# billamiable/MultiCol-SLAM-Annotation

Hardware: AMD Instinct MI355X
Metric: kfeatures/sec + LocalBA iters/sec, 3×754×480 fisheye, 1/2/4/8 MI355X (higher is better)
Workload: dtype u8; 1 GPU; config B: 3-cam Lafida rig 754x480, 2000 feat/cam, extract + consecutive-multi-frame top-2 Hamming match; parallelism=dp1 (independent multi-frame segments)

## Files before the change

multicol-slam-annotation_amd/csrc/extractor.hip:

```cpp
#include "host_util.hpp"
#include "extractor_plan.hpp"
#include "extractor_kernels.hpp"
#include "pyr_units.hpp"
#include <algorithm>
#include <cstdlib>
#include <cstring>
#include <new>
#include <vector>

namespace mcs {

template <typename T>
static int dalloc(T** p, size_t count, size_t pad_bytes = 256) {
  *p = nullptr;
  MCS_HIP_CHECK(hipMalloc((void**)p, count * sizeof(T) + pad_bytes));
  return MCS_OK;
}

}

struct mcs_extractor {
  mcs::Plan plan;
  int device = 0;
  int max_frames = 0;
  int32_t* d_xofs = nullptr; int16_t* d_alpha = nullptr;
  int32_t* d_yofs = nullptr; int16_t* d_beta = nullptr;
  mcs::CellDesc* d_cells = nullptr;
  mcs::FastUnit* d_units = nullptr;
  uint8_t* d_pyr = nullptr;
  uint8_t* d_blur = nullptr;
  uint32_t* d_slots = nullptr;
  int32_t* d_cell_counts = nullptr;
  uint32_t* d_cand = nullptr;
  int32_t* d_cnode = nullptr;
  uint32_t* d_sel = nullptr;
  int32_t* d_sel_count = nullptr;
  uint8_t* d_mask_pyr = nullptr; int n_masks = 0;
  mcs::FastUnit* d_munits = nullptr; int64_t munit_stride = 0;
  uint8_t* d_mask_single = nullptr;
  struct PyrTable {
    int fclass = 0; bool masked = false;
    mcs::PyrUnit* d_units = nullptr; int64_t mstride = 0;
    int32_t off[mcs::kMaxLevels] = {}, n[mcs::kMaxLevels] = {};
  };
  std::vector<PyrTable> pyr_tabs;
  std::vector<mcs::PyrNeed> pyr_need;
  uint8_t* d_in = nullptr;
  mcs_keypoint* d_kps = nullptr; uint8_t* d_desc = nullptr; int32_t* d_count = nullptr;
  uint8_t* d_dmask = nullptr;
  mcs_cam_model* d_cams = nullptr; int n_cams = 0;
  hipStream_t side = nullptr; hipEvent_t ev_fork = nullptr, ev_join = nullptr;
  const uint8_t* last_img0 = nullptr;
  int last_frames = 0;
  static constexpr int kRing = 256;
  bool timing = false;
  hipEvent_t* ev = nullptr;
  int ev_count = 0;
};

namespace mcs {

static void fill_level_ptrs(const Plan& pl, LevelPtrs& lp) {
  for (int l = 0; l < kMaxLevels; l++) {
    const bool v = l < pl.nlevels;
    lp.w[l] = v ? pl.lv[l].w : 0; lp.h[l] = v ? pl.lv[l].h : 0;
    lp.pitch[l] = v ? pl.lv[l].pitch : 0; lp.bpitch[l] = v ? pl.lv[l].bpitch : 0;
    lp.pyr_off[l] = v ? pl.lv[l].pyr_off : 0; lp.img_off[l] = v ? pl.lv[l].img_off : 0;
    lp.mask_off[l] = v ? pl.lv[l].mask_off : 0;
  }
}

// ... 14 lines not shown
      lists[(size_t)m * kMaxLevels + l].swap(lv[l]);
    }
  }
  int64_t stride = 0;
  for (int l = 0; l < pl.nlevels; l++) { t.off[l] = (int32_t)stride; stride += t.n[l]; }
  stride = std::max<int64_t>(stride, 1);
  std::vector<PyrUnit> all((size_t)nm * stride, PyrUnit{0, 0, 0, 0});
  for (int m = 0; m < nm; m++)
    for (int l = 0; l < pl.nlevels; l++) {
      const auto& v = lists[(size_t)m * kMaxLevels + l];
      std::copy(v.begin(), v.end(), all.begin() + (size_t)m * stride + t.off[l]);
    }
  int rc = dalloc(&t.d_units, all.size());
  if (rc) return rc;
  MCS_HIP_CHECK(hipMemcpy(t.d_units, all.data(), all.size() * sizeof(PyrUnit), hipMemcpyHostToDevice));
  t.mstride = nm > 1 ? stride : 0;
  h->pyr_tabs.push_back(t);
  *out = &h->pyr_tabs.back();
  return MCS_OK;
}

static inline void stage_mark(mcs_extractor* h, int stage, hipStream_t st) {
  if (!h->timing || h->ev_count >= mcs_extractor::kRing) return;
  (void)hipEventRecord(h->ev[h->ev_count * (MCS_EXTRACTOR_NSTAGES + 1) + stage], st);
}

static int run_batch(mcs_extractor* h, const uint8_t* d_images, int F, const uint8_t* mask_pyr,
                     const int32_t* d_mask_index, mcs_keypoint* d_kps,
                     int32_t* d_counts, uint8_t* d_desc, uint8_t* d_desc_masks,
                     const int32_t* d_cam_index, hipStream_t st) {
  const Plan& pl = h->plan;
  const int nl = pl.nlevels;
  const int64_t img0_fs = (int64_t)pl.W * pl.H;
  const bool per_mask = mask_pyr && mask_pyr == h->d_mask_pyr && h->d_munits;
  const bool orb = !pl.p.learn_masks && !pl.p.do_dbrief;
  const mcs_extractor::PyrTable* pt = nullptr;
  {
    const int rc = pyr_table(h, F, per_mask && orb && !h->pyr_need.empty(), &pt);
    if (rc) return rc;
  }
  auto pyr_args = [&](int l) {
    PyrArgs a;
    const LevelPlan& D = pl.lv[l];
    if (l == 0) {
      a.src = d_images; a.src_fstride = img0_fs; a.sw = D.w; a.sh = D.h; a.spitch = D.pitch;
      a.dst = nullptr; a.dst_fstride = 0; a.dpitch = 0;
      a.xofs = nullptr; a.alpha = nullptr; a.yofs = nullptr; a.beta = nullptr; a.simd_end = 0;
    } else {
      const LevelPlan& S = pl.lv[l - 1];
      a.src = (l == 1) ? d_images : h->d_pyr + S.pyr_off;
      a.src_fstride = (l == 1) ? img0_fs : pl.pyr_frame_bytes;
      a.sw = S.w; a.sh = S.h; a.spitch = S.pitch;
      a.dst = h->d_pyr + D.pyr_off; a.dst_fstride = pl.pyr_frame_bytes; a.dpitch = D.pitch;
      a.xofs = h->d_xofs + pl.xtab_off[l]; a.alpha = h->d_alpha + 2 * pl.xtab_off[l];
      a.yofs = h->d_yofs + pl.ytab_off[l]; a.beta = h->d_beta + 2 * pl.ytab_off[l];
      a.simd_end = D.simd_end;
    }
    a.blur = h->d_blur + D.img_off; a.blur_fstride = pl.img_frame_bytes; a.bpitch = D.bpitch;
    a.dw = D.w; a.dh = D.h;
    pyr_strips(D.w, D.h, F, a);
    a.nframes = F;
    a.units = pt->d_units + pt->off[l]; a.nunits = pt->n[l]; a.unit_mstride = pt->mstride;
    a.mask_index = pt->mstride ? d_mask_index : nullptr; a.nmasks = h->n_masks;
    return a;
  };
  FastRowArgs fa;
// ... 2 lines not shown
  fa.mask_pyr = mask_pyr; fa.mask_fstride = pl.mask_frame_bytes;
  fa.mask_index = d_mask_index;
  fa.nmasks = (mask_pyr && mask_pyr == h->d_mask_pyr) ? h->n_masks : 1;
  fa.cells = h->d_cells; fa.ncells = (int)pl.cells.size();
  fa.slots = h->d_slots; fa.slots_fstride = pl.slots_per_frame;
  fa.cell_counts = h->d_cell_counts;
  fa.threshold = std::min(std::max(pl.p.fast_threshold, 0), 255);
  fa.pattern = pl.p.fast_agast_type == 2 ? 16 : pl.p.fast_agast_type == 1 ? 12 : 8;
  fa.frame_count = d_counts;
  fa.nframes = F;
  fill_level_ptrs(pl, fa.lp);
  const bool wide = pl.scale_factor > 1.5;
  const bool use_side = !h->timing;
  if (use_side && !h->side) {
    MCS_HIP_CHECK(hipStreamCreateWithFlags(&h->side, hipStreamNonBlocking));
    MCS_HIP_CHECK(hipEventCreateWithFlags(&h->ev_fork, hipEventDisableTiming));
    MCS_HIP_CHECK(hipEventCreateWithFlags(&h->ev_join, hipEventDisableTiming));
  }
  stage_mark(h, 0, st);
  if (use_side) {
    MCS_HIP_CHECK(hipEventRecord(h->ev_fork, st));
    MCS_HIP_CHECK(hipStreamWaitEvent(h->side, h->ev_fork, 0));
    launch_pyr_blur(pyr_args(0), false, false, h->side);
    MCS_HIP_CHECK(hipEventRecord(h->ev_join, h->side));
  }
  for (int l = 1; l < nl; l++) launch_pyr_blur(pyr_args(l), true, wide, st);
  stage_mark(h, 1, st);
  if (use_side) MCS_HIP_CHECK(hipStreamWaitEvent(st, h->ev_join, 0));
  else launch_pyr_blur(pyr_args(0), false, false, st);
  stage_mark(h, 2, st);
  {
    FastRowArgs fl = fa;
    fl.units = per_mask ? h->d_munits : h->d_units;
    fl.nunits = per_mask ? (int)h->munit_stride : (int)pl.fast_units.size();
    fl.unit_mstride = per_mask ? h->munit_stride : 0;
    launch_fast_rows(fl, st);
  }
  stage_mark(h, 3, st);
  {
    OctArgs oa;
    std::memcpy(oa.lv, pl.lv, sizeof(oa.lv));
    oa.cells = h->d_cells;
    oa.cell_counts = h->d_cell_counts; oa.ncells = (int)pl.cells.size();
    oa.slots = h->d_slots; oa.slots_fstride = pl.slots_per_frame;
    oa.cand = h->d_cand; oa.cnode = h->d_cnode; oa.cand_fstride = pl.cand_per_frame;
    oa.sel = h->d_sel; oa.sel_fstride = pl.sel_per_frame;
    oa.sel_count = h->d_sel_count; oa.nlevels = nl;
    oa.frame_count = d_counts;
    oa.nframes = F;
    int maxl = 0;
    for (int l = 0; l < nl; l++) maxl = std::max(maxl, pl.lv[l].sel_cap);
    launch_octree(oa, maxl, st);
  }
  stage_mark(h, 4, st);
  {
    DescArgs da;
    std::memcpy(da.lv, pl.lv, sizeof(da.lv));
    da.nlevels = nl;
    da.img0 = d_images; da.img0_fstride = img0_fs;
    da.pyr = h->d_pyr; da.pyr_fstride = pl.pyr_frame_bytes;
    da.blur = h->d_blur; da.blur_fstride = pl.img_frame_bytes;
    da.sel = h->d_sel; da.sel_fstride = pl.sel_per_frame; da.sel_per_frame = pl.sel_per_frame;
    da.sel_count = h->d_sel_count;
    da.kps = d_kps; da.desc = d_desc; da.cap = pl.sel_per_frame; da.desc_size = pl.p.desc_size;
    da.nframes = F;
    da.mode = pl.p.learn_masks ? 2 : (pl.p.do_dbrief ? 1 : 0);
    da.do_dbrief = pl.p.do_dbrief ? 1 : 0;
// ... 29 lines not shown
  p->desc_size = 32;
}

int mcs_extractor_create(const mcs_extractor_params* p, int32_t width, int32_t height,
                         int32_t max_frames, int32_t device, mcs_extractor** out) {
  if (!p || !out || max_frames < 1) { set_error("null argument"); return MCS_ERR_ARG; }
  *out = nullptr;
  if (int rc = host::open_device(device, "extractor")) return rc;
  mcs_extractor* h = new (std::nothrow) mcs_extractor();
  if (!h) return MCS_ERR_ARG;
  int rc = build_plan(*p, width, height, h->plan);
  if (rc != MCS_OK) { delete h; return rc; }
  h->device = device;
  h->max_frames = max_frames;
  const Plan& pl = h->plan;
  const size_t F = (size_t)max_frames;
  static bool consts_done[64] = {false};
  if (device < 64 && !consts_done[device]) {
    if ((rc = upload_desc_constants()) != MCS_OK) { delete h; return rc; }
    consts_done[device] = true;
  }
#define ALLOC(ptr, n)                                  \
  do {                                                 \
    if ((rc = dalloc(&(ptr), (n))) != MCS_OK) {        \
      mcs_extractor_destroy(h);                        \
      return rc;                                       \
    }                                                  \
  } while (0)
  ALLOC(h->d_xofs, pl.xofs.size());
  ALLOC(h->d_alpha, pl.alpha.size());
  ALLOC(h->d_yofs, pl.yofs.size());
  ALLOC(h->d_beta, pl.beta.size());
  ALLOC(h->d_cells, pl.cells.size());
  ALLOC(h->d_units, pl.fast_units.size());
  ALLOC(h->d_pyr, F * pl.pyr_frame_bytes);
  ALLOC(h->d_blur, F * pl.img_frame_bytes);
  ALLOC(h->d_slots, F * pl.slots_per_frame);
  ALLOC(h->d_cell_counts, F * pl.cells.size());
  ALLOC(h->d_cand, F * pl.cand_per_frame);
  ALLOC(h->d_cnode, F * pl.cand_per_frame);
  ALLOC(h->d_sel, F * pl.sel_per_frame);
  ALLOC(h->d_sel_count, F * pl.nlevels);
  ALLOC(h->d_mask_single, pl.mask_frame_bytes);
  ALLOC(h->d_in, (size_t)width * height);
  ALLOC(h->d_kps, pl.sel_per_frame);
  ALLOC(h->d_desc, (size_t)pl.sel_per_frame * pl.p.desc_size);
  ALLOC(h->d_count, 1);
  ALLOC(h->d_dmask, (size_t)pl.sel_per_frame * pl.p.desc_size);
#undef ALLOC
  hipError_t e = hipSuccess;
  if (e == hipSuccess) e = hipMemcpy(h->d_xofs, pl.xofs.data(), pl.xofs.size() * 4, hipMemcpyHostToDevice);
  if (e == hipSuccess) e = hipMemcpy(h->d_alpha, pl.alpha.data(), pl.alpha.size() * 2, hipMemcpyHostToDevice);
  if (e == hipSuccess) e = hipMemcpy(h->d_yofs, pl.yofs.data(), pl.yofs.size() * 4, hipMemcpyHostToDevice);
  if (e == hipSuccess) e = hipMemcpy(h->d_beta, pl.beta.data(), pl.beta.size() * 2, hipMemcpyHostToDevice);
  if (e == hipSuccess) e = hipMemcpy(h->d_cells, pl.cells.data(), pl.cells.size() * sizeof(CellDesc), hipMemcpyHostToDevice);
  if (e == hipSuccess) e = hipMemcpy(h->d_units, pl.fast_units.data(), pl.fast_units.size() * sizeof(FastUnit), hipMemcpyHostToDevice);
  if (e != hipSuccess) {
    set_hip_error(e, "upload plan tables", __FILE__, __LINE__);
    mcs_extractor_destroy(h);
    return MCS_ERR_HIP;
  }
  *out = h;
  return MCS_OK;
}

void mcs_extractor_destroy(mcs_extractor* h) {
  if (!h) return;
  (void)hipSetDevice(h->device);
  void* ptrs[] = {h->d_xofs, h->d_alpha, h->d_yofs, h->d_beta, h->d_cells, h->d_units, h->d_pyr, h->d_blur,
                  h->d_slots, h->d_cell_counts, h->d_cand, h->d_cnode, h->d_sel, h->d_sel_count,
                  h->d_mask_pyr, h->d_munits, h->d_mask_single, h->d_in,
                  h->d_kps, h->d_desc, h->d_count, h->d_dmask, h->d_cams};
  for (void* p : ptrs)
    if (p) (void)hipFree(p);
  if (h->side) (void)hipStreamDestroy(h->side);
  if (h->ev_fork) (void)hipEventDestroy(h->ev_fork);
  if (h->ev_join) (void)hipEventDestroy(h->ev_join);
  for (auto& t : h->pyr_tabs)
    if (t.d_units) (void)hipFree(t.d_units);
  if (h->ev) {
    for (int i = 0; i < mcs_extractor::kRing * (MCS_EXTRACTOR_NSTAGES + 1); i++)
      (void)hipEventDestroy(h->ev[i]);
    delete[] h->ev;
  }
  delete h;
}

int mcs_extractor_enable_timing(mcs_extractor* h, int32_t enable) {
  if (!h) return MCS_ERR_ARG;
// ... 31 lines not shown

int mcs_extractor_levels(const mcs_extractor* h, int32_t* nlevels, int32_t* wh, int32_t* nfeat) {
  if (!h) return MCS_ERR_ARG;
  if (nlevels) *nlevels = h->plan.nlevels;
  for (int l = 0; l < h->plan.nlevels; l++) {
    if (wh) { wh[2 * l] = h->plan.lv[l].w; wh[2 * l + 1] = h->plan.lv[l].h; }
    if (nfeat) nfeat[l] = h->plan.lv[l].nfeat;
  }
  return MCS_OK;
}

int mcs_extractor_set_masks_device(mcs_extractor* h, const uint8_t* d_masks, int32_t n_masks,
                                   void* stream) {
  if (!h || n_masks < 0 || (n_masks > 0 && !d_masks)) return MCS_ERR_ARG;
  MCS_HIP_CHECK(hipSetDevice(h->device));
  if (h->d_mask_pyr) { MCS_HIP_CHECK(hipFree(h->d_mask_pyr)); h->d_mask_pyr = nullptr; }
  if (h->d_munits) { MCS_HIP_CHECK(hipFree(h->d_munits)); h->d_munits = nullptr; }
  h->n_masks = 0;
  h->munit_stride = 0;
  for (auto it = h->pyr_tabs.begin(); it != h->pyr_tabs.end();) {
    if (it->masked) { MCS_HIP_CHECK(hipFree(it->d_units)); it = h->pyr_tabs.erase(it); }
    else ++it;
  }
  h->pyr_need.clear();
  if (n_masks == 0) return MCS_OK;
  const Plan& pl = h->plan;
  int rc = dalloc(&h->d_mask_pyr, (size_t)n_masks * pl.mask_frame_bytes);
  if (rc) return rc;
  launch_mask_pyramids(pl, d_masks, n_masks, h->d_mask_pyr, (hipStream_t)stream);
  MCS_HIP_CHECK(hipGetLastError());
  std::vector<uint8_t> hm((size_t)n_masks * pl.mask_frame_bytes);
  MCS_HIP_CHECK(hipStreamSynchronize((hipStream_t)stream));
  MCS_HIP_CHECK(hipMemcpy(hm.data(), h->d_mask_pyr, hm.size(), hipMemcpyDeviceToHost));
  std::vector<std::vector<FastUnit>> lists(n_masks);
  std::vector<PyrNeed> need(n_masks);
  size_t stride = 0;
  for (int m = 0; m < n_masks; m++) {
    std::vector<FastUnit> dead;
    build_masked_units(pl, hm.data() + (size_t)m * pl.mask_frame_bytes, lists[m], dead);
    build_pyr_need(pl, hm.data() + (size_t)m * pl.mask_frame_bytes, lists[m], need[m]);
    lists[m].insert(lists[m].end(), dead.begin(), dead.end());
    stride = std::max(stride, lists[m].size());
  }
  stride = std::max<size_t>(stride, 1);
  FastUnit pad{};
  std::vector<FastUnit> all((size_t)n_masks * stride, pad);
  for (int m = 0; m < n_masks; m++) std::copy(lists[m].begin(), lists[m].end(), all.begin() + (size_t)m * stride);
  if ((rc = dalloc(&h->d_munits, all.size())) != MCS_OK) return rc;
  MCS_HIP_CHECK(hipMemcpy(h->d_munits, all.data(), all.size() * sizeof(FastUnit), hipMemcpyHostToDevice));
  h->munit_stride = (int64_t)stride;
  h->n_masks = n_masks;
  h->pyr_need.swap(need);
  return MCS_OK;
}

int mcs_extractor_set_cam_models(mcs_extractor* h, const mcs_cam_model* models, int32_t n) {
  if (!h || n < 0 || (n > 0 && !models)) return MCS_ERR_ARG;
  for (int i = 0; i < n; i++)
    if (models[i].p_deg < 1 || models[i].p_deg > 16 || models[i].invp_deg < 1 ||
        models[i].invp_deg > 16) {
      set_error("camera polynomial length must be 1..16");
      return MCS_ERR_ARG;
    }
  MCS_HIP_CHECK(hipSetDevice(h->device));
  if (h->d_cams) { MCS_HIP_CHECK(hipFree(h->d_cams)); h->d_cams = nullptr; }
  h->n_cams = 0;
  if (n == 0) return MCS_OK;
  int rc = dalloc(&h->d_cams, (size_t)n);
  if (rc) return rc;
  MCS_HIP_CHECK(hipMemcpy(h->d_cams, models, sizeof(mcs_cam_model) * n, hipMemcpyHostToDevice));
  h->n_cams = n;
  return MCS_OK;
}

int mcs_extract_batch_device_ex(mcs_extractor* h, const uint8_t* d_images, int32_t n_frames,
                                const int32_t* d_cam_index, mcs_keypoint* d_kps,
                                int32_t* d_counts, uint8_t* d_desc, uint8_t* d_desc_masks,
                                void* stream) {
  if (!h || !d_images || !d_kps || !d_counts || !d_desc || n_frames < 1) {
    set_error("null argument"); return MCS_ERR_ARG;
  }
  if (n_frames > h->max_frames) { set_error("n_frames > max_frames"); return MCS_ERR_CAPACITY; }
// ... 114 lines not shown
```

multicol-slam-annotation_amd/csrc/extractor_kernels.hpp:

```cpp
#pragma once
#include <algorithm>
#include <hip/hip_runtime.h>
#include <cstdint>
#include "extractor_plan.hpp"
#include "pyr_units.hpp"

namespace mcs {

__device__ __forceinline__ bool xcd_frame_map(int b, int F, int items, int* frame, int* item) {
  const int x = b & 7, k = b >> 3;
  const int f = x + 8 * (k / items);
  *item = k % items;
  *frame = f;
  return f < F;
}
inline unsigned xcd_grid(int F, int items) { return (unsigned)(8 * ((F + 7) / 8) * items); }

struct LevelPtrs {
  int32_t w[kMaxLevels], h[kMaxLevels], pitch[kMaxLevels], bpitch[kMaxLevels];
  int64_t pyr_off[kMaxLevels], img_off[kMaxLevels], mask_off[kMaxLevels];
};

struct PyrArgs {
  const uint8_t* src; int64_t src_fstride; int sw, sh, spitch;
  uint8_t* dst; int64_t dst_fstride; int dpitch;
  uint8_t* blur; int64_t blur_fstride; int bpitch;
  int dw, dh;
  const int32_t* xofs; const int16_t* alpha; const int32_t* yofs; const int16_t* beta;
  int simd_end;
  int nframes;
  const PyrUnit* units; int nunits; int64_t unit_mstride;
  const int32_t* mask_index; int nmasks;
  int tiles_x, tiles_y;
  int core, seg_rows;
};
inline void pyr_strips(int dw, int dh, int F, PyrArgs& a) {
  pyr_strip_geometry(dw, dh, F, &a.core, &a.tiles_x, &a.seg_rows, &a.tiles_y);
}
void launch_pyr_blur(const PyrArgs& a, bool resize, bool wide, hipStream_t st);

void launch_mask_pyramids(const Plan& pl, const uint8_t* d_masks, int n, uint8_t* dst,
                          hipStream_t st);
struct FastRowArgs {
  const uint8_t* img0; int64_t img0_fstride;
  const uint8_t* pyr; int64_t pyr_fstride;
  const uint8_t* mask_pyr; int64_t mask_fstride;
  const int32_t* mask_index; int nmasks;
  const FastUnit* units; int nunits;
  int64_t unit_mstride;
  const CellDesc* cells; int ncells;
  uint32_t* slots; int64_t slots_fstride;
  int32_t* cell_counts;
  int threshold;
  uint32_t kk, rbits;
  int pattern;
  int32_t* frame_count;
  int nframes;
  LevelPtrs lp;
};
void launch_fast_rows(const FastRowArgs& a, hipStream_t st);

struct OctArgs {
  LevelPlan lv[kMaxLevels];
  const CellDesc* cells;
  const int32_t* cell_counts; int ncells;
  const uint32_t* slots; int64_t slots_fstride;
  uint32_t* cand; int32_t* cnode; int64_t cand_fstride;
  uint32_t* sel; int64_t sel_fstride;
  int32_t* sel_count; int nlevels;
  int32_t* frame_count;
  int nframes;
};
void launch_octree(const OctArgs& a, int max_list, hipStream_t st);

struct DescArgs {
  LevelPlan lv[kMaxLevels];
  int nlevels;
  const uint8_t* img0; int64_t img0_fstride;
  const uint8_t* pyr; int64_t pyr_fstride;
  const uint8_t* blur; int64_t blur_fstride;
  const uint32_t* sel; int64_t sel_fstride; int sel_per_frame;
// ... 12 lines not shown
```

multicol-slam-annotation_amd/csrc/extractor_plan.cpp:

```cpp
#include "extractor_plan.hpp"
#include "common.hpp"
#include <algorithm>
#include <cmath>
#include <cstdio>

namespace mcs {

namespace {

int16_t sat_s16_from_float(float v) {
  int i = cv_roundf(v);
  return (int16_t)std::min(std::max(i, -32768), 32767);
}

void linear_tables(int sw, int sh, int dw, int dh, Plan& pl) {
  const double scale_x = 1. / ((double)dw / sw), scale_y = 1. / ((double)dh / sh);
  for (int dx = 0; dx < dw; dx++) {
    float fx = (float)((dx + 0.5) * scale_x - 0.5);
    int sx = cv_floorf(fx);
    fx -= sx;
    if (sx < 0) { fx = 0; sx = 0; }
    if (sx + 1 >= sw && sx >= sw - 1) { fx = 0; sx = sw - 1; }
    pl.xofs.push_back(sx);
    pl.alpha.push_back(sat_s16_from_float((1.f - fx) * 2048));
// ... 21 lines not shown
    bool ok = true;
    for (int a = c; a < e && ok; a += per) ok = fits(a, std::min(e, a + per));
    if (!ok) continue;
    for (int a = c; a < e; a += per) {
      const int b = std::min(e, a + per);
      FastUnit u;
      u.level = (int16_t)level; u.ncells = (int16_t)(b - a);
      u.wy0 = cells[a].wy0; u.wy1 = cells[a].wy1;
      u.ux0 = cells[a].wx0; u.ux1 = cells[b - 1].wx1;
      u.xa = (int16_t)((u.ux0 - 3) & ~3);
      u.wcell = (int16_t)wcell;
      u.cell0 = a;
      out.push_back(u);
    }
    return;
  }
}

void zero_runs(const std::vector<CellDesc>& cells, int c, int e, int level, int wcell,
               std::vector<FastUnit>& out) {
  for (int a = c; a < e; a += 64) {
    const int b = std::min(e, a + 64);
    FastUnit u;
    u.level = (int16_t)level; u.ncells = (int16_t)(b - a);
    u.wy0 = u.wy1 = cells[a].wy0;
    u.ux0 = cells[a].wx0; u.ux1 = cells[b - 1].wx1;
    u.xa = (int16_t)((u.ux0 - 3) & ~3);
    u.wcell = (int16_t)wcell;
    u.cell0 = a;
    out.push_back(u);
  }
}

}

int build_plan(const mcs_extractor_params& p, int W, int H, Plan& pl) {
  if (W <= 0 || H <= 0 || p.nlevels < 1 || p.nlevels > kMaxLevels || p.nfeatures < 0 ||
      !(p.scale_factor > 1.0f)) {
    set_error("invalid extractor parameters: width, height > 0, nfeatures >= 0, nlevels in 1..12 "
              "and scale_factor in (1, 2.2] are required");
    return MCS_ERR_ARG;
  }
  if (!((double)p.scale_factor <= kMaxScaleFactor)) {
    set_error("scale_factor > 2.2f exceeds the pyramid kernel's source tile (accepted: 1 < "
              "scale_factor <= 2.2f)");
    return MCS_ERR_UNSUPPORTED;
  }
  if (p.desc_size != 16 && p.desc_size != 32 && p.desc_size != 64) {
    set_error("desc_size must be 16, 32 or 64 (src/cTracking.cpp:133)");
    return MCS_ERR_ARG;
  }
  if (p.use_agast) {
    set_error("AGAST (useAgast != 0) is not implemented; FAST types 0, 1, 2 are");
    return MCS_ERR_UNSUPPORTED;
  }
  if (p.fast_agast_type < 0 || p.fast_agast_type > 2) {
    set_error("fastAgastType must be 0 (TYPE_5_8), 1 (TYPE_7_12) or 2 (TYPE_9_16)");
    return MCS_ERR_ARG;
  }
  pl.p = p;
  pl.W = W; pl.H = H; pl.nlevels = p.nlevels;
  pl.scale_factor = (double)p.scale_factor;

  double sf[kMaxLevels], isf[kMaxLevels];
  sf[0] = 1; isf[0] = 1;
  for (int i = 1; i < p.nlevels; i++) sf[i] = sf[i - 1] * pl.scale_factor;
// ... 88 lines not shown
    L.cand_cap = slot - L.cand_off;
    pl.unit_begin[l] = (int32_t)pl.fast_units.size();
    L.wcell = wCell;
    for (int c = L.cell_begin; c < L.cell_end;) {
      int e = c;
      while (e < L.cell_end && pl.cells[e].wy0 == pl.cells[c].wy0) e++;
      split_runs(pl.cells, c, e, l, wCell, pl.fast_units);
      c = e;
    }
    pl.max_cells_level = std::max(pl.max_cells_level, L.cell_end - L.cell_begin);
    if (L.cell_end - L.cell_begin > kMaxCellsPerLevel) {
      set_error("too many FAST cells in one level");
      return MCS_ERR_UNSUPPORTED;
    }

    L.width_rel = maxBX - kMinBorder;
    L.height_rel = maxBY - kMinBorder;
    L.nini = cv_round((double)L.width_rel / L.height_rel);
    if (L.nini < 1) {
      set_error("octree nIni == 0 (level taller than 2x its width): reference indexes out of range");
      return MCS_ERR_UNSUPPORTED;
    }
    L.hx = (double)L.width_rel / L.nini;
    const int cap = (std::max(L.nfeat + 3, 4 * L.nini) + 1) & ~1;
    if (cap > kOctMaxL) {
      set_error("per-level feature budget exceeds the octree kernel's node bound (1024)");
      return MCS_ERR_UNSUPPORTED;
    }
    L.sel_off = sel;
    L.sel_cap = cap;
    sel += cap;
  }
  for (int l = p.nlevels; l <= kMaxLevels; l++) pl.unit_begin[l] = (int32_t)pl.fast_units.size();
  pl.pyr_frame_bytes = pyr_off;
  pl.img_frame_bytes = img_off;
  pl.mask_frame_bytes = mask_off;
  pl.slots_per_frame = slot;
  pl.cand_per_frame = slot;
  pl.sel_per_frame = sel;
  return MCS_OK;
}

void build_masked_units(const Plan& pl, const uint8_t* mask_pyr, std::vector<FastUnit>& live,
                        std::vector<FastUnit>& dead) {
  for (int l = 0; l < pl.nlevels; l++) {
    const LevelPlan& L = pl.lv[l];
    const uint8_t* m = mask_pyr + L.mask_off;
    auto cell_live = [&](const CellDesc& cd) {
      for (int y = cd.wy0; y < cd.wy1; y++)
        for (int x = cd.wx0; x < cd.wx1; x++)
          if (m[(int64_t)y * L.bpitch + x]) return true;
      return false;
    };
    for (int c = L.cell_begin; c < L.cell_end;) {
      int e = c;
      while (e < L.cell_end && pl.cells[e].wy0 == pl.cells[c].wy0) e++;
      int a0 = -1, a1 = -1;
      for (int k = c; k < e; k++)
        if (cell_live(pl.cells[k])) { if (a0 < 0) a0 = k; a1 = k + 1; }
      if (a0 < 0) {
        zero_runs(pl.cells, c, e, l, L.wcell, dead);
      } else {
        zero_runs(pl.cells, c, a0, l, L.wcell, dead);
        split_runs(pl.cells, a0, a1, l, L.wcell, live);
        zero_runs(pl.cells, a1, e, l, L.wcell, dead);
      }
// ... 7 lines not shown
```

multicol-slam-annotation_amd/csrc/extractor_plan.hpp:

```cpp
#pragma once
#include <cstdint>
#include <vector>
#include "../../include/mcs_extractor.h"

namespace mcs {

constexpr int kMaxLevels = 12;
constexpr int kEdgeThreshold = 25;
constexpr int kMinBorder = kEdgeThreshold - 3;
constexpr int kPatchSize = 32;
constexpr int kHalfPatch = 16;
constexpr int kMaxCellDim = 64;
constexpr int kMaxCellsPerLevel = 2048;
constexpr int kOctMaxL = 1024;
constexpr double kMaxScaleFactor = (double)2.2f;

struct CellDesc {
  int32_t level;
  int16_t wx0, wy0, wx1, wy1;
  int32_t slot_off;
  int32_t slot_cap;
};

struct FastUnit {
  int16_t level, ncells;
  int16_t wy0, wy1;
  int16_t ux0, ux1;
  int16_t xa, wcell;
  int32_t cell0;
};
constexpr int kFastUnitSpan = 252;

struct LevelPlan {
  int32_t w, h;
  int32_t pitch;
  int32_t bpitch;
  int64_t pyr_off;
  int64_t img_off;
  int64_t mask_off;
  int32_t cell_begin, cell_end;
  int32_t cand_off, cand_cap;
  int32_t sel_off, sel_cap;
  int32_t nfeat;
  int32_t nini;
  double hx;
  int32_t width_rel, height_rel;
  int32_t simd_end;
  int32_t wcell;
  int32_t patch_size_scaled;
  float scale;
};

struct Plan {
  mcs_extractor_params p;
  int32_t W = 0, H = 0, nlevels = 0;
  double scale_factor = 1.2;
  LevelPlan lv[kMaxLevels];
  std::vector<CellDesc> cells;
  std::vector<FastUnit> fast_units;
  int32_t unit_begin[kMaxLevels + 1] = {};
  int64_t pyr_frame_bytes = 0;
  int64_t img_frame_bytes = 0;
  int64_t mask_frame_bytes = 0;
  int32_t slots_per_frame = 0;
  int32_t cand_per_frame = 0;
  int32_t sel_per_frame = 0;
  int32_t max_cells_level = 0;
  int32_t max_win_w = 0, max_win_h = 0;
  std::vector<int32_t> xofs, yofs;
  std::vector<int16_t> alpha, beta;
  std::vector<int64_t> xtab_off, ytab_off;
};

int build_plan(const mcs_extractor_params& p, int W, int H, Plan& plan);

void build_masked_units(const Plan& pl, const uint8_t* mask_pyr, std::vector<FastUnit>& live,
                        std::vector<FastUnit>& dead);

}
```

multicol-slam-annotation_amd/csrc/k_fast_rows.hip:

```cpp
#include "common.hpp"
#include "extractor_kernels.hpp"

namespace mcs {

#ifdef MCS_FAST_PROBE
__device__ unsigned long long g_fast_probe[8];
extern "C" int mcs_debug_fast_probe(unsigned long long* out, int reset) {
  if (hipMemcpyFromSymbol(out, HIP_SYMBOL(g_fast_probe), sizeof(g_fast_probe)) != hipSuccess) return -1;
  if (reset) {
    unsigned long long z[8] = {0, 0, 0, 0, 0, 0, 0, 0};
    if (hipMemcpyToSymbol(HIP_SYMBOL(g_fast_probe), z, sizeof(z)) != hipSuccess) return -1;
  }
  return 0;
}
#define FP_BEGIN() unsigned long long acc_[8] = {0, 0, 0, 0, 0, 0, 0, 0}; \
  const long long t_begin_ = __builtin_amdgcn_s_memtime()
#define FP_T(v) const long long v = __builtin_amdgcn_s_memtime()
#define FP_ADD(k, v) (acc_[k] += (unsigned long long)(v))
#define FP_END() do { FP_ADD(4, __builtin_amdgcn_s_memtime() - t_begin_); \
    if (lane == 0) for (int k = 0; k < 8; k++) atomicAdd(&g_fast_probe[k], acc_[k]); } while (0)
#else
#define FP_BEGIN() do { } while (0)
#define FP_T(v) do { } while (0)
#define FP_ADD(k, v) do { } while (0)
#define FP_END() do { } while (0)
#endif

namespace {
#ifndef MCS_FAST_BAND
#define MCS_FAST_BAND 5
#endif
constexpr int kBand = MCS_FAST_BAND;
static_assert(kBand >= 3 && kBand <= 8, "band height");
constexpr int kScoreRows = kBand + 3;
constexpr int kRingBytes = (kBand + 6) * 256, kScoreBytes = kScoreRows * 256;
constexpr int kListCap = 248 + kBand * 248;
constexpr int kScoreBase = 4 * kRingBytes, kListBase = kScoreBase + 4 * kScoreBytes;
constexpr int kLdsBytes = kListBase + 4 * 2 * (kListCap + 2);

typedef _Float16 h2 __attribute__((ext_vector_type(2)));
typedef unsigned short u16x2 __attribute__((ext_vector_type(2)));
__device__ __forceinline__ h2 hmin3(h2 a, h2 b, h2 c) {
  return __builtin_elementwise_minimum(__builtin_elementwise_minimum(a, b), c);
}
__device__ __forceinline__ h2 hmax3(h2 a, h2 b, h2 c) {
  return __builtin_elementwise_maximum(__builtin_elementwise_maximum(a, b), c);
}

__device__ __forceinline__ int fr_max3(int a, int b, int c) { return max(max(a, b), c); }

template <int P>
__device__ __forceinline__ int fast_small(const uint8_t* lds, uint32_t ring_base, int e, int t) {
  constexpr int K = P / 2;
  constexpr int c12[12][2] = {{0, 2}, {1, 2}, {2, 1}, {2, 0}, {2, -1}, {1, -2},
                              {0, -2}, {-1, -2}, {-2, -1}, {-2, 0}, {-2, 1}, {-1, 2}};
  constexpr int c8[8][2] = {{0, 1}, {1, 1}, {1, 0}, {1, -1}, {0, -1}, {-1, -1}, {-1, 0}, {-1, 1}};
  auto at = [&](int dx, int dy) -> int {
    return lds[ring_base + (uint32_t)(e + dy * 256 + dx)];
  };
  const int v = at(0, 0);
  int d[P];
#pragma unroll
  for (int k = 0; k < P; k++) d[k] = v - (P == 12 ? at(c12[k][0], c12[k][1]) : at(c8[k % 8][0], c8[k % 8][1]));
  auto tb = [&](int k) -> int { const int q = d[k % P]; return (q > t ? 1 : 0) | (q < -t ? 2 : 0); };
  const int qd = (tb(0) | tb(8)) & (tb(2) | tb(10)) & (tb(4) | tb(12)) & (tb(6) | tb(14)) &
                 (tb(1) | tb(9)) & (tb(3) | tb(11)) & (tb(5) | tb(13)) & (tb(7) | tb(15));
  int dark = -256, bright = -256;
#pragma unroll
  for (int k = 0; k < P; k++) {
    int mn = d[k], mxv = d[k];
#pragma unroll
    for (int j = 1; j <= K; j++) { mn = min(mn, d[(k + j) % P]); mxv = max(mxv, d[(k + j) % P]); }
    dark = max(dark, mn);
    bright = max(bright, -mxv);
  }
  const bool corner = ((qd & 1) && dark > t) || ((qd & 2) && bright > t);
  return corner ? max(max(t, dark), bright) : 0;
}
}

template <int PAT>
__global__ __launch_bounds__(256) void k_fast_rows(FastRowArgs a) {
  __shared__ __attribute__((aligned(16))) uint8_t lds[kLdsBytes];
  const int wv = __builtin_amdgcn_readfirstlane(threadIdx.x >> 6), lane = threadIdx.x & 63;
  const uint32_t ring_base = (uint32_t)wv * kRingBytes;
  const uint32_t sc_base = kScoreBase + (uint32_t)wv * kScoreBytes;
  uint32_t* const ring32 = reinterpret_cast<uint32_t*>(lds + ring_base);
  uint8_t* const sc8 = lds + sc_base;
  uint16_t* const list = reinterpret_cast<uint16_t*>(lds + kListBase + wv * 2 * (kListCap + 2));
  uint32_t raw_rel = 0, sc_rel = 0;
  auto sc_at = [&](int e, int dy, int dx) -> uint8_t& {
    return lds[sc_rel + (uint32_t)(e + dy * 256 + dx)];
  };
  int f, item;
  if (!xcd_frame_map(blockIdx.x, a.nframes, (a.nunits + 3) / 4, &f, &item)) return;
  const int ui = item * 4 + wv;
  if (ui >= a.nunits) return;
  auto zero_count = [&] { if (ui == 0 && lane == 0) a.frame_count[f] = 0; };
  const int mi = a.mask_index ? min(max(a.mask_index[f], 0), a.nmasks - 1) : 0;
  const FastUnit u = a.units[(int64_t)mi * a.unit_mstride + ui];
  FP_BEGIN();
  const int level = u.level, nc = u.ncells, wh = u.wy1 - u.wy0;
  int32_t* const cnt_out = a.cell_counts + (int64_t)f * a.ncells + u.cell0;
  if (wh <= 0) {
    if (lane < nc) cnt_out[lane] = 0;
    zero_count();
    return;
  }
  const uint8_t* const mrow0 =
      a.mask_pyr ? a.mask_pyr + (int64_t)mi * a.mask_fstride +
                       a.lp.mask_off[level] + (int64_t)(u.wy0 - 3) * a.lp.bpitch[level] + u.xa
                 : nullptr;
  const int mpitch = a.lp.bpitch[level];
  const int t = a.threshold;
  const int xa = u.xa, wc = u.wcell, span = u.ux1 - u.ux0;
  const uint32_t magic = 65536u / (uint32_t)wc + 1u;
  const int pitch = a.lp.pitch[level];
  const uint8_t* const img = (level == 0) ? a.img0 + (int64_t)f * a.img0_fstride
                                          : a.pyr + (int64_t)f * a.pyr_fstride + a.lp.pyr_off[level];
  const uint8_t* const row0 = img + (int64_t)(u.wy0 - 3) * pitch + xa;

  uint32_t detm = 0;
#pragma unroll
  for (int k = 0; k < 4; k++) {
    const int x = xa + 4 * lane + k;
    detm |= (x >= u.ux0 && x < u.ux1) ? (0x80u << (8 * k)) : 0u;
  }
  const int slot_off = lane < nc ? a.cells[u.cell0 + lane].slot_off : 0;
  uint32_t* const outf = a.slots + (int64_t)f * a.slots_fstride;
  int cnt = 0;

  auto load_row = [&](int r) -> uint32_t {
    return dev::align_down4(row0 + r * pitch)[lane];
  };
  auto fix_row = [&](int r, uint32_t own) -> uint32_t {
    const uint32_t sh = (uint32_t)((uintptr_t)(row0 + r * pitch) & 3);
    const uint32_t nxt = (uint32_t)__builtin_amdgcn_mov_dpp((int)own, 0x130 , 0xF, 0xF, true);
    return __builtin_amdgcn_alignbyte(nxt, own, sh);
  };
  auto load_mrow = [&](int r) -> uint32_t {
    if (!mrow0) return 0xFFFFFFFFu;
    return reinterpret_cast<const uint32_t*>(mrow0 + r * mpitch)[lane];
  };

#pragma unroll
  for (int i = 0; i < kScoreRows; i++) *reinterpret_cast<uint32_t*>(sc8 + 256 * i + 4 * lane) = 0u;
  uint32_t w[6];
#pragma unroll
  for (int i = 0; i < 6; i++) w[i] = load_row(i);
  uint32_t pf[kBand];
#pragma unroll
  for (int i = 0; i < kBand; i++) pf[i] = load_row(6 + i);
  uint32_t m[kBand + 2], mpf[kBand];
#pragma unroll
  for (int i = 0; i < kBand + 2; i++) m[i] = load_mrow(2 + i);
#pragma unroll
  for (int i = 0; i < kBand; i++) mpf[i] = load_mrow(kBand + 4 + i);
#pragma unroll
  for (int i = 0; i < 6; i++) w[i] = fix_row(i, w[i]);

  const int nbands = (wh + kBand - 1) / kBand;
  int ncarry = 0;
  FP_ADD(7, __builtin_amdgcn_s_memtime() - t_begin_);
  for (int b = 0; b < nbands; b++) {
    FP_T(t0_);
    const int y0 = 3 + b * kBand, y1 = min(y0 + kBand, 3 + wh);
    uint32_t rows[6 + kBand];
#pragma unroll
    for (int i = 0; i < 6; i++) rows[i] = w[i];
#pragma unroll
    for (int i = 0; i < kBand; i++) rows[6 + i] = fix_row(y0 + 3 + i, pf[i]);
    if (b > 0) {
#pragma unroll
      for (int i = 0; i < 2; i++) m[i] = m[kBand + i];
#pragma unroll
// ... 134 lines not shown
          const h2 x3 = 3 * k + 2 < n ? amx[3 * k + 2] : x1, y3 = 3 * k + 2 < n ? amn[3 * k + 2] : y1v;
          amx[k] = hmin3(x1, x2, x3);
          amn[k] = hmax3(y1v, y2, y3);
        }
      }
      const uint32_t bmx = __builtin_bit_cast(uint32_t, amx[0]), bmn = __builtin_bit_cast(uint32_t, amn[0]);
      const int dark_a = va - (int)(bmx & 0xFFFFu), dark_b = vb - (int)(bmx >> 16);
      const int bright_a = (int)(bmn & 0xFFFFu) - va, bright_b = (int)(bmn >> 16) - vb;
      const bool ca = ja < ns && (dark_a > t || bright_a > t);
      const bool cb = jb < ns && (dark_b > t || bright_b > t);
      if (ca) sc_at(ea, 0, 0) = (uint8_t)max(max(t, dark_a), bright_a);
      if (cb) sc_at(eb, 0, 0) = (uint8_t)max(max(t, dark_b), bright_b);
      const uint64_t bal_a = __ballot(ca);
      if (ca) list[ncorn + __popcll(bal_a & lt)] = (uint16_t)ea;
      ncorn += __popcll(bal_a);
      const uint64_t bal_b = __ballot(cb);
      if (cb) list[ncorn + __popcll(bal_b & lt)] = (uint16_t)eb;
      ncorn += __popcll(bal_b);
      nlast += __popcll(__ballot(ca && (ea >> 8) == y1 - 1)) + __popcll(__ballot(cb && (eb >> 8) == y1 - 1));
    }
    dev::wave_sync();
    FP_T(t3_);
    FP_ADD(2, t3_ - t2_);

    const bool last_band = b + 1 == nbands;
    const int nproc = last_band ? ncorn : ncorn - nlast;
    for (int j0 = 0; j0 < nproc; j0 += 64) {
      const int j = j0 + lane;
      bool keep = false;
      int k = 0;
      uint32_t rec = 0;
      if (j < nproc) {
        const int e = list[j], y = e >> 8, x = e & 0xFF;
        const int cx = xa + x - u.ux0;
        k = (int)(((uint32_t)cx * magic) >> 16);
        const int cs = k * wc, ce = min(cs + wc, span);
        auto sv = [&](int dy, int dx) -> int { return sc_at(e, dy, dx); };
        const int e0 = sv(0, 0);
        int mx = max(sv(-1, 0), sv(1, 0));
        if (cx > cs) mx = max(mx, fr_max3(sv(-1, -1), sv(0, -1), sv(1, -1)));
        if (cx + 1 < ce) mx = max(mx, fr_max3(sv(-1, 1), sv(0, 1), sv(1, 1)));
        keep = e0 >= 2 && e0 > mx;
        rec = (uint32_t)(xa + x - kMinBorder) | ((uint32_t)(u.wy0 + y - 3 - kMinBorder) << 12) |
              ((uint32_t)(e0 - 1) << 24);
      }
      {
        const int e = list[min(j, nproc - 1)];
        const int ri = ((e >> 8) & 0x7F) - (y0 - 1), x = e & 0xFF;
        uint32_t mw = 0;
#pragma unroll
        for (int i = 0; i <= kBand; i++) {
          const uint32_t mi = (uint32_t)__builtin_amdgcn_ds_bpermute((x >> 2) << 2, (int)m[i]);
          mw = ri == i ? mi : mw;
        }
        keep = keep && ((mw >> (8 * (x & 3))) & 0xFFu) != 0;
      }
      uint64_t bk = __ballot(keep);
      while (bk) {
        const int kc = __builtin_amdgcn_readlane(k, (int)__builtin_ctzll(bk));
        const bool mine = keep && k == kc;
        const uint64_t bm = __ballot(mine);
        const int base = __builtin_amdgcn_readlane(cnt, kc) + __builtin_amdgcn_readlane(slot_off, kc);
        if (mine) outf[base + __popcll(bm & lt)] = rec;
        if (lane == kc) cnt += __popcll(bm);
        bk &= ~bm;
      }
    }
    ncarry = 0;
    if (!last_band && nlast > 0) {
      uint32_t v[4];
#pragma unroll
      for (int i = 0; i < 4; i++) {
        const int jj = lane + 64 * i;
        v[i] = jj < nlast ? list[nproc + jj] : 0u;
      }
      dev::wave_sync();
#pragma unroll
      for (int i = 0; i < 4; i++) {
        const int jj = lane + 64 * i;
        if (jj < nlast) list[jj] = (uint16_t)v[i];
      }
      ncarry = nlast;
    }
    dev::wave_sync();
    FP_T(t4_);
    FP_ADD(3, t4_ - t3_);
  }
  if (lane < nc) cnt_out[lane] = cnt;
  zero_count();
  FP_END();
}

void launch_fast_rows(const FastRowArgs& a_in, hipStream_t st) {
  FastRowArgs a = a_in;
  const int t = a.threshold;
  const uint32_t r = (uint32_t)(t & 1), K = (uint32_t)(t + 256 + (int)r) / 2;
  a.rbits = r * 0x01010101u;
  a.kk = (K <= 255 ? (~(K - 1) & 0xFFu) : 0u) * 0x01010101u;
  const unsigned g = xcd_grid(a.nframes, (a.nunits + 3) / 4);
  if (a.pattern == 12) hipLaunchKernelGGL(k_fast_rows<12>, dim3(g), dim3(256), 0, st, a);
  else if (a.pattern == 8) hipLaunchKernelGGL(k_fast_rows<8>, dim3(g), dim3(256), 0, st, a);
  else hipLaunchKernelGGL(k_fast_rows<16>, dim3(g), dim3(256), 0, st, a);
}

}
```

Before: 476,500 kfeatures/s.

## Pack two FAST cell runs into each 64-lane wave to fill idle lanes

Adds a host-side packer that merges pairs of FAST work units (cell runs sharing level, window height and 4-byte row alignment) into a single FastWave, with a lane split between two runs. The FAST row kernel now computes per-lane offsets, detection masks, cell indices and record bases from whichever run a lane belongs to. The aim is to cut partially idle waves and the total number of waves launched for the FAST stage. In exchange the kernel does more per-lane address arithmetic, the list capacity grows, and a new 4-byte alignment precondition on input images is enforced.

```diff
diff --git a/multicol-slam-annotation_amd/csrc/extractor.hip b/multicol-slam-annotation_amd/csrc/extractor.hip
--- a/multicol-slam-annotation_amd/csrc/extractor.hip
+++ b/multicol-slam-annotation_amd/csrc/extractor.hip
@@ -26,7 +26,7 @@
   int32_t* d_xofs = nullptr; int16_t* d_alpha = nullptr;
   int32_t* d_yofs = nullptr; int16_t* d_beta = nullptr;
   mcs::CellDesc* d_cells = nullptr;
-  mcs::FastUnit* d_units = nullptr;
+  mcs::FastWave* d_units = nullptr;
   uint8_t* d_pyr = nullptr;
   uint8_t* d_blur = nullptr;
   uint32_t* d_slots = nullptr;
@@ -36,7 +36,7 @@
   uint32_t* d_sel = nullptr;
   int32_t* d_sel_count = nullptr;
   uint8_t* d_mask_pyr = nullptr; int n_masks = 0;
-  mcs::FastUnit* d_munits = nullptr; int64_t munit_stride = 0;
+  mcs::FastWave* d_munits = nullptr; int64_t munit_stride = 0;
   uint8_t* d_mask_single = nullptr;
   struct PyrTable {
     int fclass = 0; bool masked = false;
@@ -117,6 +117,10 @@
   const Plan& pl = h->plan;
   const int nl = pl.nlevels;
   const int64_t img0_fs = (int64_t)pl.W * pl.H;
+  if (pl.W % 4 == 0 && ((uintptr_t)d_images & 3) != 0) {
+    set_error("images must be 4-byte aligned when the width is a multiple of 4");
+    return MCS_ERR_ARG;
+  }
   const bool per_mask = mask_pyr && mask_pyr == h->d_mask_pyr && h->d_munits;
   const bool orb = !pl.p.learn_masks && !pl.p.do_dbrief;
   const mcs_extractor::PyrTable* pt = nullptr;
@@ -185,7 +189,7 @@
   {
     FastRowArgs fl = fa;
     fl.units = per_mask ? h->d_munits : h->d_units;
-    fl.nunits = per_mask ? (int)h->munit_stride : (int)pl.fast_units.size();
+    fl.nunits = per_mask ? (int)h->munit_stride : (int)pl.fast_waves.size();
     fl.unit_mstride = per_mask ? h->munit_stride : 0;
     launch_fast_rows(fl, st);
   }
@@ -281,7 +285,7 @@
   ALLOC(h->d_yofs, pl.yofs.size());
   ALLOC(h->d_beta, pl.beta.size());
   ALLOC(h->d_cells, pl.cells.size());
-  ALLOC(h->d_units, pl.fast_units.size());
+  ALLOC(h->d_units, pl.fast_waves.size());
   ALLOC(h->d_pyr, F * pl.pyr_frame_bytes);
   ALLOC(h->d_blur, F * pl.img_frame_bytes);
   ALLOC(h->d_slots, F * pl.slots_per_frame);
@@ -303,7 +307,7 @@
   if (e == hipSuccess) e = hipMemcpy(h->d_yofs, pl.yofs.data(), pl.yofs.size() * 4, hipMemcpyHostToDevice);
   if (e == hipSuccess) e = hipMemcpy(h->d_beta, pl.beta.data(), pl.beta.size() * 2, hipMemcpyHostToDevice);
   if (e == hipSuccess) e = hipMemcpy(h->d_cells, pl.cells.data(), pl.cells.size() * sizeof(CellDesc), hipMemcpyHostToDevice);
-  if (e == hipSuccess) e = hipMemcpy(h->d_units, pl.fast_units.data(), pl.fast_units.size() * sizeof(FastUnit), hipMemcpyHostToDevice);
+  if (e == hipSuccess) e = hipMemcpy(h->d_units, pl.fast_waves.data(), pl.fast_waves.size() * sizeof(FastWave), hipMemcpyHostToDevice);
   if (e != hipSuccess) {
     set_hip_error(e, "upload plan tables", __FILE__, __LINE__);
     mcs_extractor_destroy(h);
@@ -401,22 +405,23 @@
   std::vector<uint8_t> hm((size_t)n_masks * pl.mask_frame_bytes);
   MCS_HIP_CHECK(hipStreamSynchronize((hipStream_t)stream));
   MCS_HIP_CHECK(hipMemcpy(hm.data(), h->d_mask_pyr, hm.size(), hipMemcpyDeviceToHost));
-  std::vector<std::vector<FastUnit>> lists(n_masks);
+  std::vector<std::vector<FastWave>> lists(n_masks);
   std::vector<PyrNeed> need(n_masks);
   size_t stride = 0;
   for (int m = 0; m < n_masks; m++) {
-    std::vector<FastUnit> dead;
-    build_masked_units(pl, hm.data() + (size_t)m * pl.mask_frame_bytes, lists[m], dead);
-    build_pyr_need(pl, hm.data() + (size_t)m * pl.mask_frame_bytes, lists[m], need[m]);
-    lists[m].insert(lists[m].end(), dead.begin(), dead.end());
+    std::vector<FastUnit> live, dead;
+    build_masked_units(pl, hm.data() + (size_t)m * pl.mask_frame_bytes, live, dead);
+    build_pyr_need(pl, hm.data() + (size_t)m * pl.mask_frame_bytes, live, need[m]);
+    live.insert(live.end(), dead.begin(), dead.end());
+    pack_fast_units(pl, live, lists[m]);
     stride = std::max(stride, lists[m].size());
   }
   stride = std::max<size_t>(stride, 1);
-  FastUnit pad{};
-  std::vector<FastUnit> all((size_t)n_masks * stride, pad);
+  FastWave pad{};
+  std::vector<FastWave> all((size_t)n_masks * stride, pad);
   for (int m = 0; m < n_masks; m++) std::copy(lists[m].begin(), lists[m].end(), all.begin() + (size_t)m * stride);
   if ((rc = dalloc(&h->d_munits, all.size())) != MCS_OK) return rc;
-  MCS_HIP_CHECK(hipMemcpy(h->d_munits, all.data(), all.size() * sizeof(FastUnit), hipMemcpyHostToDevice));
+  MCS_HIP_CHECK(hipMemcpy(h->d_munits, all.data(), all.size() * sizeof(FastWave), hipMemcpyHostToDevice));
   h->munit_stride = (int64_t)stride;
   h->n_masks = n_masks;
   h->pyr_need.swap(need);
diff --git a/multicol-slam-annotation_amd/csrc/extractor_kernels.hpp b/multicol-slam-annotation_amd/csrc/extractor_kernels.hpp
--- a/multicol-slam-annotation_amd/csrc/extractor_kernels.hpp
+++ b/multicol-slam-annotation_amd/csrc/extractor_kernels.hpp
@@ -46,7 +46,7 @@
   const uint8_t* pyr; int64_t pyr_fstride;
   const uint8_t* mask_pyr; int64_t mask_fstride;
   const int32_t* mask_index; int nmasks;
-  const FastUnit* units; int nunits;
+  const FastWave* units; int nunits;
   int64_t unit_mstride;
   const CellDesc* cells; int ncells;
   uint32_t* slots; int64_t slots_fstride;
diff --git a/multicol-slam-annotation_amd/csrc/extractor_plan.cpp b/multicol-slam-annotation_amd/csrc/extractor_plan.cpp
--- a/multicol-slam-annotation_amd/csrc/extractor_plan.cpp
+++ b/multicol-slam-annotation_amd/csrc/extractor_plan.cpp
@@ -77,6 +77,76 @@
   }
 }
 
+FastRun make_run(const std::vector<CellDesc>& cells, int a, int b) {
+  FastRun r;
+  r.wy0 = cells[a].wy0;
+  r.ux0 = cells[a].wx0; r.ux1 = cells[b - 1].wx1;
+  r.ncells = (int16_t)(b - a);
+  r.cell0 = a;
+  return r;
+}
+
+}
+
+int fast_run_lanes(const Plan& pl, int level, int ux0, int ux1) {
+  const int xa = (ux0 - 3) & ~3;
+  return (ux1 + 3 - xa + 3) / 4 + (pl.lv[level].pitch % 4 != 0 ? 1 : 0);
+}
+
+void pack_fast_units(const Plan& pl, const std::vector<FastUnit>& units, std::vector<FastWave>& out) {
+  const std::vector<CellDesc>& cells = pl.cells;
+  auto lanes = [&](int level, int a, int b) {
+    return fast_run_lanes(pl, level, cells[a].wx0, cells[b - 1].wx1);
+  };
+  auto take = [&](int level, int a, int e, int room) {
+    int b = a;
+    while (b < e && lanes(level, a, b + 1) <= room) b++;
+    return b;
+  };
+  auto open_wave = [&](const FastUnit& u, int wh, const FastRun& r0) {
+    FastWave w;
+    w.level = u.level; w.wcell = u.wcell; w.wh = (int16_t)wh; w.split = kFastWaveLanes;
+    w.r[0] = r0;
+    w.r[1] = r0; w.r[1].ncells = 0; w.r[1].ux1 = r0.ux0;
+    out.push_back(w);
+  };
+  int open = -1, used = 0;
+  for (size_t i = 0; i < units.size();) {
+    const FastUnit& u = units[i];
+    if (u.wy1 <= u.wy0) {
+      FastRun r;
+      r.wy0 = u.wy0; r.ux0 = u.ux0; r.ux1 = u.ux1;
+      r.ncells = u.ncells; r.cell0 = u.cell0;
+      open_wave(u, 0, r);
+      open = -1;
+      i++;
+      continue;
+    }
+    size_t j = i;
+    int e = u.cell0;
+    while (j < units.size() && units[j].level == u.level && units[j].wy0 == u.wy0 &&
+           units[j].wy1 == u.wy1 && units[j].cell0 == e) { e += units[j].ncells; j++; }
+    int c = u.cell0;
+    const int wh = u.wy1 - u.wy0;
+    if (open >= 0 && out[open].level == u.level && out[open].wh == wh &&
+        (u.wy0 - out[open].r[0].wy0) * pl.lv[u.level].pitch % 4 == 0) {
+      const int b = take(u.level, c, e, kFastWaveLanes - used);
+      if (b > c) {
+        out[open].split = (int16_t)used;
+        out[open].r[1] = make_run(cells, c, b);
+        c = b;
+      }
+    }
+    open = -1;
+    while (c < e) {
+      const int b = take(u.level, c, e, kFastWaveLanes);
+      open_wave(u, wh, make_run(cells, c, b));
+      used = lanes(u.level, c, b);
+      open = used < kFastWaveLanes ? (int)out.size() - 1 : -1;
+      c = b;
+    }
+    i = j;
+  }
 }
 
 int build_plan(const mcs_extractor_params& p, int W, int H, Plan& pl) {
@@ -231,6 +301,8 @@
     sel += cap;
   }
   for (int l = p.nlevels; l <= kMaxLevels; l++) pl.unit_begin[l] = (int32_t)pl.fast_units.size();
+  pl.fast_waves.clear();
+  pack_fast_units(pl, pl.fast_units, pl.fast_waves);
   pl.pyr_frame_bytes = pyr_off;
   pl.img_frame_bytes = img_off;
   pl.mask_frame_bytes = mask_off;
diff --git a/multicol-slam-annotation_amd/csrc/extractor_plan.hpp b/multicol-slam-annotation_amd/csrc/extractor_plan.hpp
--- a/multicol-slam-annotation_amd/csrc/extractor_plan.hpp
+++ b/multicol-slam-annotation_amd/csrc/extractor_plan.hpp
@@ -31,6 +31,21 @@
 };
 constexpr int kFastUnitSpan = 252;
 
+struct FastRun {
+  int16_t wy0;
+  int16_t ux0, ux1;
+  int16_t ncells;
+  int32_t cell0;
+};
+struct FastWave {
+  int16_t level, wcell;
+  int16_t wh;
+  int16_t split;
+  FastRun r[2];
+};
+static_assert(sizeof(FastWave) == 32, "read as eight dwords");
+constexpr int kFastWaveLanes = 64;
+
 struct LevelPlan {
   int32_t w, h;
   int32_t pitch;
@@ -58,6 +73,7 @@
   LevelPlan lv[kMaxLevels];
   std::vector<CellDesc> cells;
   std::vector<FastUnit> fast_units;
+  std::vector<FastWave> fast_waves;
   int32_t unit_begin[kMaxLevels + 1] = {};
   int64_t pyr_frame_bytes = 0;
   int64_t img_frame_bytes = 0;
@@ -77,4 +93,8 @@
 void build_masked_units(const Plan& pl, const uint8_t* mask_pyr, std::vector<FastUnit>& live,
                         std::vector<FastUnit>& dead);
 
+int fast_run_lanes(const Plan& pl, int level, int ux0, int ux1);
+
+void pack_fast_units(const Plan& pl, const std::vector<FastUnit>& units, std::vector<FastWave>& out);
+
 }
diff --git a/multicol-slam-annotation_amd/csrc/k_fast_rows.hip b/multicol-slam-annotation_amd/csrc/k_fast_rows.hip
--- a/multicol-slam-annotation_amd/csrc/k_fast_rows.hip
+++ b/multicol-slam-annotation_amd/csrc/k_fast_rows.hip
@@ -34,7 +34,7 @@
 static_assert(kBand >= 3 && kBand <= 8, "band height");
 constexpr int kScoreRows = kBand + 3;
 constexpr int kRingBytes = (kBand + 6) * 256, kScoreBytes = kScoreRows * 256;
-constexpr int kListCap = 248 + kBand * 248;
+constexpr int kListCap = 256 + kBand * 256;
 constexpr int kScoreBase = 4 * kRingBytes, kListBase = kScoreBase + 4 * kScoreBytes;
 constexpr int kLdsBytes = kListBase + 4 * 2 * (kListCap + 2);
 
@@ -98,40 +98,58 @@
   if (ui >= a.nunits) return;
   auto zero_count = [&] { if (ui == 0 && lane == 0) a.frame_count[f] = 0; };
   const int mi = a.mask_index ? min(max(a.mask_index[f], 0), a.nmasks - 1) : 0;
-  const FastUnit u = a.units[(int64_t)mi * a.unit_mstride + ui];
+  const FastWave u = a.units[(int64_t)mi * a.unit_mstride + ui];
   FP_BEGIN();
-  const int level = u.level, nc = u.ncells, wh = u.wy1 - u.wy0;
-  int32_t* const cnt_out = a.cell_counts + (int64_t)f * a.ncells + u.cell0;
+  const int level = u.level, wh = u.wh;
+  const int ncA = u.r[0].ncells, nc = ncA + u.r[1].ncells;
+  const int cell_l = lane < ncA ? u.r[0].cell0 + lane : u.r[1].cell0 + (lane - ncA);
+  int32_t* const cnt_out = a.cell_counts + (int64_t)f * a.ncells;
   if (wh <= 0) {
-    if (lane < nc) cnt_out[lane] = 0;
+    if (lane < nc) cnt_out[cell_l] = 0;
     zero_count();
     return;
   }
-  const uint8_t* const mrow0 =
-      a.mask_pyr ? a.mask_pyr + (int64_t)mi * a.mask_fstride +
-                       a.lp.mask_off[level] + (int64_t)(u.wy0 - 3) * a.lp.bpitch[level] + u.xa
-                 : nullptr;
+  const int split = u.split, split4 = 4 * split;
+  const bool in_b = lane >= split;
+  const int xoA = (u.r[0].ux0 - 3) & ~3, xoB = ((u.r[1].ux0 - 3) & ~3) - split4;
+  const int xl = (in_b ? xoB : xoA) + 4 * lane;
   const int mpitch = a.lp.bpitch[level];
   const int t = a.threshold;
-  const int xa = u.xa, wc = u.wcell, span = u.ux1 - u.ux0;
+  const int wc = u.wcell;
   const uint32_t magic = 65536u / (uint32_t)wc + 1u;
   const int pitch = a.lp.pitch[level];
   const uint8_t* const img = (level == 0) ? a.img0 + (int64_t)f * a.img0_fstride
                                           : a.pyr + (int64_t)f * a.pyr_fstride + a.lp.pyr_off[level];
-  const uint8_t* const row0 = img + (int64_t)(u.wy0 - 3) * pitch + xa;
+  const int dy = u.r[1].wy0 - u.r[0].wy0;
+  const uint8_t* const row0 = img + (int64_t)(u.r[0].wy0 - 3) * pitch + xoA;
+  const uint32_t lb = 4u * (uint32_t)lane + (in_b ? (uint32_t)(dy * pitch + xoB - xoA) : 0u);
+  const uint8_t* const mrow0 =
+      a.mask_pyr ? a.mask_pyr + (int64_t)mi * a.mask_fstride +
+                       a.lp.mask_off[level] + (int64_t)(u.r[0].wy0 - 3) * mpitch + xoA
+                 : nullptr;
+  const uint32_t mlb = 4u * (uint32_t)lane + (in_b ? (uint32_t)(dy * mpitch + xoB - xoA) : 0u);
 
   uint32_t detm = 0;
-#pragma unroll
-  for (int k = 0; k < 4; k++) {
-    const int x = xa + 4 * lane + k;
-    detm |= (x >= u.ux0 && x < u.ux1) ? (0x80u << (8 * k)) : 0u;
+  {
+    const int ux0l = in_b ? u.r[1].ux0 : u.r[0].ux0, ux1l = in_b ? u.r[1].ux1 : u.r[0].ux1;
+#pragma unroll
+    for (int k = 0; k < 4; k++) {
+      const int x = xl + k;
+      detm |= (x >= ux0l && x < ux1l) ? (0x80u << (8 * k)) : 0u;
+    }
   }
-  const int slot_off = lane < nc ? a.cells[u.cell0 + lane].slot_off : 0;
+  const int slot_off = lane < nc ? a.cells[cell_l].slot_off : 0;
   uint32_t* const outf = a.slots + (int64_t)f * a.slots_fstride;
   int cnt = 0;
+  const int cxoA = xoA - u.r[0].ux0, cxoB = xoB - u.r[1].ux0;
+  const int spanA = u.r[0].ux1 - u.r[0].ux0, spanB = u.r[1].ux1 - u.r[1].ux0;
+  const int recA = (xoA - kMinBorder) + ((u.r[0].wy0 - 3 - kMinBorder) << 12);
+  const int recB = (xoB - kMinBorder) + ((u.r[1].wy0 - 3 - kMinBorder) << 12);
 
   auto load_row = [&](int r) -> uint32_t {
-    return dev::align_down4(row0 + r * pitch)[lane];
+    uint32_t o = lb;
+    asm volatile("" : "+v"(o));
+    return *reinterpret_cast<const uint32_t*>(reinterpret_cast<const uint8_t*>(dev::align_down4(row0 + r * pitch)) + o);
   };
   auto fix_row = [&](int r, uint32_t own) -> uint32_t {
     const uint32_t sh = (uint32_t)((uintptr_t)(row0 + r * pitch) & 3);
@@ -140,7 +158,7 @@
   };
   auto load_mrow = [&](int r) -> uint32_t {
     if (!mrow0) return 0xFFFFFFFFu;
-    return reinterpret_cast<const uint32_t*>(mrow0 + r * mpitch)[lane];
+    return *reinterpret_cast<const uint32_t*>(mrow0 + r * mpitch + mlb);
   };
 
 #pragma unroll
@@ -341,17 +359,18 @@
       uint32_t rec = 0;
       if (j < nproc) {
         const int e = list[j], y = e >> 8, x = e & 0xFF;
-        const int cx = xa + x - u.ux0;
+        const bool eb = x >= split4;
+        const int cx = (eb ? cxoB : cxoA) + x;
         k = (int)(((uint32_t)cx * magic) >> 16);
-        const int cs = k * wc, ce = min(cs + wc, span);
+        const int cs = k * wc, ce = min(cs + wc, eb ? spanB : spanA);
+        k += eb ? ncA : 0;
         auto sv = [&](int dy, int dx) -> int { return sc_at(e, dy, dx); };
         const int e0 = sv(0, 0);
         int mx = max(sv(-1, 0), sv(1, 0));
         if (cx > cs) mx = max(mx, fr_max3(sv(-1, -1), sv(0, -1), sv(1, -1)));
         if (cx + 1 < ce) mx = max(mx, fr_max3(sv(-1, 1), sv(0, 1), sv(1, 1)));
         keep = e0 >= 2 && e0 > mx;
-        rec = (uint32_t)(xa + x - kMinBorder) | ((uint32_t)(u.wy0 + y - 3 - kMinBorder) << 12) |
-              ((uint32_t)(e0 - 1) << 24);
+        rec = (uint32_t)((eb ? recB : recA) + x + (y << 12)) | ((uint32_t)(e0 - 1) << 24);
       }
       {
         const int e = list[min(j, nproc - 1)];
@@ -395,7 +414,7 @@
     FP_T(t4_);
     FP_ADD(3, t4_ - t3_);
   }
-  if (lane < nc) cnt_out[lane] = cnt;
+  if (lane < nc) cnt_out[cell_l] = cnt;
   zero_count();
   FP_END();
 }
```

Result: faster. 482,500 kfeatures/s (median of 6 runs) (+1.2%).
